# liuzm-slam/VLOAM-NOTED

Measured on NVIDIA B200. Metric: scans/sec, higher is better.
Workload: dtype f32+f64

## Files before the change

vloam-noted_b200/csrc/capi.cu:

```cuda
#include <stdlib.h>
#include <string>
#include <vector>
#include "common.cuh"

static bool g_capture_default = false;
bool vl_debug_capture(const vloam_b200_ctx* c) { return c->h_vScalars && c->h_vScalars[0] != 0; }
int vl_lm_rescan_sorted(vloam_b200_ctx* c);
int vl_solver_trace(vloam_b200_ctx* c, long long* out16);
int vl_lo_trace(vloam_b200_ctx* c, int* out, int n);
int vl_sr_trace(vloam_b200_ctx* c, long long* out, int n);

extern "C" {

void vloam_b200_default_params(vloam_b200_params* p) {
  p->n_scans = 64; p->minimum_range = 5.0f; p->line_res = 0.4f; p->plane_res = 0.8f; p->mapping_skip_frame = 1; p->reserved = 0;
}

const char* vloam_b200_last_error(const vloam_b200_ctx* c) { return c ? c->err : "null context"; }

#define VL_CUDA_CREATE(call)                                                                                       \
  do {                                                                                                             \
    cudaError_t e_ = (call);                                                                                       \
    if (e_ != cudaSuccess) { fprintf(stderr, "vloam_b200_create: %s: %s\n", #call, cudaGetErrorString(e_)); return VLOAM_E_CUDA; } \
  } while (0)

static int alloc_sr_fixed(vloam_b200_ctx* c) {
  const int R = VL_MAX_RINGS, S = VL_MAX_RINGS * VL_SECTORS;
  VL_CUDA_CREATE(cudaEventCreateWithFlags(&c->evSR, cudaEventDisableTiming));
  VL_CUDA_CREATE(cudaEventCreateWithFlags(&c->evSRfeat, cudaEventDisableTiming));
  VL_CUDA_CREATE(cudaMalloc(&c->ringCount, sizeof(int) * R));
  VL_CUDA_CREATE(cudaMalloc(&c->ringStart, sizeof(int) * (R + 1)));
  VL_CUDA_CREATE(cudaMemset(c->ringCount, 0, sizeof(int) * R));
  VL_CUDA_CREATE(cudaMemset(c->ringStart, 0, sizeof(int) * (R + 1)));
  VL_CUDA_CREATE(cudaMalloc(&c->srs, sizeof(SrScalars)));
  VL_CUDA_CREATE(cudaMemset(c->srs, 0, sizeof(SrScalars)));
  VL_CUDA_CREATE(cudaMallocHost(&c->h_srs, sizeof(SrScalars)));
  memset(c->h_srs, 0, sizeof(SrScalars));
  VL_CUDA_CREATE(cudaMalloc(&c->provSharp, sizeof(int) * S * 2));
  VL_CUDA_CREATE(cudaMalloc(&c->provLess, sizeof(int) * S * 20));
  VL_CUDA_CREATE(cudaMalloc(&c->provFlat, sizeof(int) * S * 4));
  int** smalls[] = {&c->cntSharp, &c->cntLess, &c->cntFlat, &c->offSharp, &c->offLess, &c->offFlat};
  for (int** q : smalls) { VL_CUDA_CREATE(cudaMalloc(q, sizeof(int) * S)); VL_CUDA_CREATE(cudaMemset(*q, 0, sizeof(int) * S)); }
  VL_CUDA_CREATE(cudaMalloc(&c->ringDsCount, sizeof(int) * R));
  VL_CUDA_CREATE(cudaMalloc(&c->ringDsOff, sizeof(int) * R));
  c->sr_counts_valid = false; c->n_in = 0; c->nKept = c->nSharp = c->nLessSharp = c->nFlat = c->nLessFlat = 0;
  return VLOAM_OK;
}
static void free_sr_set(vloam_b200_ctx* c) {
  void* dev[] = {c->ringCount, c->ringStart, c->srs, c->provSharp, c->provLess, c->provFlat, c->cntSharp, c->cntLess, c->cntFlat, c->offSharp,
                 c->offLess, c->offFlat, c->ringDsCount, c->ringDsOff, c->in.p, c->ring.p, c->ori.p, c->blockHist.p, c->cloud.p, c->curv.p,
                 c->label.p, c->picked.p, c->sortScratch.p, c->lessFlatProv.p, c->selIdx.p, c->sharp.p, c->flat.p};
  for (void* p : dev) vl_dev_free(c, p);
  if (c->h_srs) cudaFreeHost(c->h_srs);
  if (c->evSR) cudaEventDestroy(c->evSR);
  if (c->evSRfeat) cudaEventDestroy(c->evSRfeat);
}

static int create_impl(vloam_b200_ctx* c, const vloam_b200_params* p, int device);

int vloam_b200_create(const vloam_b200_params* p, int device, vloam_b200_ctx** out) {
  if (!p || !out) return VLOAM_E_INVALID;
  *out = nullptr;
  if (p->n_scans != 16 && p->n_scans != 32 && p->n_scans != 64 && p->n_scans != 128) return VLOAM_E_INVALID;
  if (!(p->line_res >= 0.05f) || !(p->plane_res >= 0.05f) || p->mapping_skip_frame < 1) return VLOAM_E_INVALID;
  if (p->reserved & ~(VLOAM_FLAG_DISTORTION | VLOAM_FLAG_TRANSFORM_TO_END)) return VLOAM_E_INVALID;
  VL_CUDA_CREATE(cudaSetDevice(device));
  vloam_b200_ctx* c = new vloam_b200_ctx();
  const int r = create_impl(c, p, device);
  if (r != VLOAM_OK) { vloam_b200_destroy(c); (void)cudaGetLastError(); return r; }
  *out = c;
  return VLOAM_OK;
}

static int create_impl(vloam_b200_ctx* c, const vloam_b200_params* p, int device) {
  c->prm = *p; c->device = device; c->err[0] = 0; c->launches = 0; c->worker = nullptr; c->timing = false; c->cur = 0;
  c->sr_counts_valid = false; c->n_in = 0; c->lo_inited = false; c->lo_frameCount = 0; c->lm_frameCount = 0; c->lm_optimized = 0; c->skip_frame = false;
  c->nKept = c->nSharp = c->nLessSharp = c->nFlat = c->nLessFlat = 0; c->nCornerLast = c->nSurfLast = 0;
  c->cornerLastPtr = nullptr; c->surfLastPtr = nullptr;
  for (int k = 0; k < 4; ++k) c->dbgLoCost[k] = c->dbgLmCost[k] = 0;
  for (int k = 0; k < 3; ++k) c->stage_ms[k] = 0;
  c->prof_name[0] = 0; c->prof_n = 0; c->prof_created = 0; c->prof_bytes = 0; c->prof_next_bytes = 0;
  {
    const char* e = getenv("VLOAM_ARENA_MB");
    const size_t mb = e ? (size_t)max(atoll(e), 0LL) : 1024;
    c->arena = nullptr; c->arenaCap = 0; c->arenaTop = 0;
    if (mb) { VL_CUDA_CREATE(cudaMalloc(&c->arena, mb << 20)); c->arenaCap = mb << 20; }
  }
  cudaDeviceProp prop;
  VL_CUDA_CREATE(cudaGetDeviceProperties(&prop, device));
  c->num_sms = prop.multiProcessorCount;
  int prLow = 0, prHigh = 0;
  VL_CUDA_CREATE(cudaDeviceGetStreamPriorityRange(&prLow, &prHigh));
  int lv[4] = {2, 1, 2, 2};
  int lvLO = 2;
  if (const char* e = getenv("VLOAM_PRIO")) sscanf(e, "%d,%d,%d,%d,%d", &lv[0], &lv[1], &lv[2], &lv[3], &lvLO);
  if (getenv("VLOAM_NO_PRIORITIES")) lv[0] = lv[1] = lv[2] = lv[3] = lvLO = 0;
  int pr[5];
  for (int k = 0; k < 4; ++k) pr[k] = max(prLow - lv[k], prHigh);
  pr[4] = max(prLow - lvLO, prHigh);
  VL_CUDA_CREATE(cudaStreamCreateWithPriority(&c->stream, cudaStreamNonBlocking, pr[0]));
  VL_CUDA_CREATE(cudaStreamCreateWithPriority(&c->stream2, cudaStreamNonBlocking, pr[1]));
  VL_CUDA_CREATE(cudaStreamCreateWithPriority(&c->stream3, cudaStreamNonBlocking, pr[2]));
  VL_CUDA_CREATE(cudaStreamCreateWithPriority(&c->stream4, cudaStreamNonBlocking, pr[1]));
  VL_CUDA_CREATE(cudaEventCreateWithFlags(&c->evStacksC, cudaEventDisableTiming));
  VL_CUDA_CREATE(cudaStreamCreateWithPriority(&c->streamAux, cudaStreamNonBlocking, pr[2]));
  VL_CUDA_CREATE(cudaEventCreateWithFlags(&c->evAux, cudaEventDisableTiming));
  VL_CUDA_CREATE(cudaEventCreateWithFlags(&c->evAuxZero, cudaEventDisableTiming));
  VL_CUDA_CREATE(cudaEventCreateWithFlags(&c->evUpd, cudaEventDisableTiming));
  VL_CUDA_CREATE(cudaEventCreateWithFlags(&c->evStacks, cudaEventDisableTiming));
  VL_CUDA_CREATE(cudaEventCreateWithFlags(&c->evLast, cudaEventDisableTiming));
  VL_CUDA_CREATE(cudaEventCreateWithFlags(&c->evPose, cudaEventDisableTiming));
  VL_CUDA_CREATE(cudaEventCreateWithFlags(&c->evMap, cudaEventDisableTiming));
  VL_CUDA_CREATE(cudaEventCreateWithFlags(&c->evKeys, cudaEventDisableTiming));
  for (int k = 0; k < 2; ++k) VL_CUDA_CREATE(cudaEventCreateWithFlags(&c->evKeysSel[k], cudaEventDisableTiming));
  c->stacksReady = false; c->lm_reset_pending = true; c->lastSet = 0; c->loGridValid[0] = c->loGridValid[1] = false;
  for (int k = 0; k < 4; ++k) VL_CUDA_CREATE(cudaEventCreate(&c->ev[k]));
  for (int k = 0; k < 12; ++k) { VL_CUDA_CREATE(cudaEventCreate(&c->evx[k])); VL_CUDA_CREATE(cudaEventRecord(c->evx[k], c->stream)); }
  VL_TRY(alloc_sr_fixed(c));
  c->srNext = new SrSet();
  vl_sr_swap(c, *c->srNext);
  { const int r_ = alloc_sr_fixed(c); vl_sr_swap(c, *c->srNext); if (r_ != VLOAM_OK) return r_; }
  c->srNext2 = new SrSet();
  vl_sr_swap(c, *c->srNext2);
  { const int r_ = alloc_sr_fixed(c); vl_sr_swap(c, *c->srNext2); if (r_ != VLOAM_OK) return r_; }
  c->srNextKey = c->srNext2Key = nullptr; c->srNextValid = c->srNext2Valid = false; c->srPendCount = 0;
  VL_CUDA_CREATE(cudaStreamCreateWithPriority(&c->streamSR, cudaStreamNonBlocking, pr[3]));
  VL_CUDA_CREATE(cudaMalloc(&c->los, sizeof(LoScalars)));
  VL_CUDA_CREATE(cudaMalloc(&c->losNext, sizeof(LoScalars)));
  VL_CUDA_CREATE(cudaEventCreateWithFlags(&c->evS2, cudaEventDisableTiming));
  VL_CUDA_CREATE(cudaMallocHost(&c->h_s2flag, 64)); *c->h_s2flag = 0; c->s2seq = 0;
  VL_CUDA_CREATE(cudaEventCreateWithFlags(&c->evLoSolve, cudaEventDisableTiming));
  VL_CUDA_CREATE(cudaEventCreateWithFlags(&c->evLoNext, cudaEventDisableTiming));
  VL_CUDA_CREATE(cudaEventCreateWithFlags(&c->evEnd, cudaEventDisableTiming));
  VL_CUDA_CREATE(cudaStreamCreateWithPriority(&c->streamLO, cudaStreamNonBlocking, pr[4]));
  c->loNextValid = c->loNextQueued = c->srAdopted = c->s2Done = false; c->loAssumeMonotone = c->inProcessFrame = c->loDeferred = false; c->srDeferred = c->sideSubmitted = false; c->preDeferred = c->loPreValid = c->sideWaitsIssued = c->earlyLoArmed = c->stacksAdopted = false; c->loNextSet = 0; c->stackSel = 0; c->stacksNextReady = false;
  VL_CUDA_CREATE(cudaMallocHost(&c->h_los, sizeof(LoScalars)));
  LoScalars hl; memset(&hl, 0, sizeof hl); hl.para_q[3] = 1.0; hl.q_w[3] = 1.0;
  VL_CUDA_CREATE(cudaMemcpy(c->los, &hl, sizeof hl, cudaMemcpyHostToDevice));
  *c->h_los = hl;
  VL_CUDA_CREATE(cudaMalloc(&c->loRingTbl, sizeof(int) * 4 * 160));
  VL_CUDA_CREATE(cudaMalloc(&c->evalOut, sizeof(EvalOut)));
  VL_CUDA_CREATE(cudaMalloc(&c->lms, sizeof(LmSolveState)));
  VL_CUDA_CREATE(cudaMemset(c->lms, 0, sizeof(LmSolveState)));
  VL_CUDA_CREATE(cudaMallocHost(&c->h_lms, sizeof(LmSolveState)));
  VL_CUDA_CREATE(cudaMalloc(&c->lmm, sizeof(LmScalars)));
  VL_CUDA_CREATE(cudaMallocHost(&c->h_lmm, sizeof(LmScalars)));
  memset(c->h_lmm, 0, sizeof(LmScalars));
  VL_CUDA_CREATE(cudaMalloc(&c->cubeC, sizeof(MapCubeTable)));
  VL_CUDA_CREATE(cudaMalloc(&c->cubeS, sizeof(MapCubeTable)));
  VL_CUDA_CREATE(cudaMalloc(&c->vScalars, sizeof(int) * 256));
  VL_CUDA_CREATE(cudaMemset(c->vScalars, 0, sizeof(int) * 256));
  VL_CUDA_CREATE(cudaMallocHost(&c->h_vScalars, sizeof(int) * 256));
  memset(c->h_vScalars, 0, sizeof(int) * 256);
  c->h_vScalars[0] = g_capture_default ? 1 : 0;
  int r = vl_lm_init(c);
  if (r == VLOAM_OK) r = vl_sr_set_attrs(c);
  if (r == VLOAM_OK) r = vl_sort_set_attrs(c);
  if (r == VLOAM_OK) r = vl_solver_set_attrs(c);
  if (r == VLOAM_OK) r = vl_lo_preload(c);
  if (r == VLOAM_OK) r = vl_vg_preload(c);
  if (r == VLOAM_OK) r = vl_lm_preload(c);
  if (r != VLOAM_OK) { fprintf(stderr, "vloam_b200_create: %s\n", c->err); return r; }
  VL_CUDA_CREATE(cudaDeviceSynchronize());
  return VLOAM_OK;
}

void vloam_b200_destroy(vloam_b200_ctx* c) {
  if (!c) return;
  cudaSetDevice(c->device);
  vl_lm_shutdown(c);
  cudaStreamSynchronize(c->stream); cudaStreamSynchronize(c->stream2); cudaStreamSynchronize(c->stream3); cudaStreamSynchronize(c->stream4);
  cudaStreamSynchronize(c->streamSR);
  free_sr_set(c);
  if (c->srNext) { vl_sr_swap(c, *c->srNext); free_sr_set(c); delete c->srNext; c->srNext = nullptr; }
  if (c->srNext2) { vl_sr_swap(c, *c->srNext2); free_sr_set(c); delete c->srNext2; c->srNext2 = nullptr; }
  cudaStreamDestroy(c->streamSR);
  vl_lm_free(c);
  vl_scan_free(&c->loScan[0]); vl_scan_free(&c->loScan[1]);
  if (c->streamLO) { cudaStreamSynchronize(c->streamLO); cudaStreamDestroy(c->streamLO); }
  cudaEventDestroy(c->evS2); cudaEventDestroy(c->evLoSolve); cudaEventDestroy(c->evLoNext); if (c->evEnd) cudaEventDestroy(c->evEnd);
  void* singles[] = {c->los, c->losNext, c->evalOut, c->lms, c->lmm, c->cubeC, c->cubeS, c->vScalars, c->loRingTbl, c->loGridCells[0].p, c->loGridCells[1].p,
                     c->loGridCellOf.p, c->loGridSorted[0].p, c->loGridSorted[1].p, c->dbgLoCorner[0].p, c->dbgLoCorner[1].p, c->dbgLoSurf[0].p,
                     c->dbgLoSurf[1].p, c->dbgKnnIdx[0][0].p, c->dbgKnnIdx[0][1].p, c->dbgKnnIdx[1][0].p, c->dbgKnnIdx[1][1].p, c->dbgKnnD2[0][0].p,
                     c->dbgKnnD2[0][1].p, c->dbgKnnD2[1][0].p, c->dbgKnnD2[1][1].p, c->dbgKnnOk[0][0].p, c->dbgKnnOk[0][1].p, c->dbgKnnOk[1][0].p,
                     c->dbgKnnOk[1][1].p};
  for (void* p : singles) vl_dev_free(c, p);
  void* bufs[] = {c->lessSharp[0].p, c->lessSharp[1].p, c->lessSharp[2].p, c->lessFlat[0].p, c->lessFlat[1].p, c->lessFlat[2].p, c->endSharp[0].p, c->endSharp[1].p, c->endSharp[2].p, c->endFlat[0].p, c->endFlat[1].p, c->endFlat[2].p, c->loCornerIdx.p, c->loSurfIdx.p, c->factors.p, c->factorS.p, c->factorValid.p, c->loFactors.p, c->loFactorValid.p, c->evalPartials.p,
                  c->poolC.p, c->poolS.p, c->stackC.p, c->stackS.p, c->stackCN.p, c->stackSN.p, c->fromMapC.p, c->fromMapS.p, c->knnIdx.p, c->knnD2.p, c->knnOk.p,
                  c->vKeys.p, c->vKeys2.p, c->vHead.p, c->vScan.p, c->vScan2.p, c->vOut.p, c->vIn.p, c->regOut.p, c->tailKeys.p, c->staging.p};
  for (void* p : bufs) vl_dev_free(c, p);
  if (c->h_s2flag) cudaFreeHost(c->h_s2flag);
  cudaFreeHost(c->h_los); cudaFreeHost(c->h_lms); cudaFreeHost(c->h_lmm); cudaFreeHost(c->h_vScalars);
  for (int k = 0; k < 4; ++k) cudaEventDestroy(c->ev[k]);
  for (int k = 0; k < 12; ++k) cudaEventDestroy(c->evx[k]);
  cudaStreamSynchronize(c->stream2); cudaStreamSynchronize(c->stream3);
  cudaEventDestroy(c->evStacks); cudaEventDestroy(c->evLast); cudaEventDestroy(c->evPose); cudaEventDestroy(c->evMap); cudaEventDestroy(c->evKeys); cudaEventDestroy(c->evKeysSel[0]); cudaEventDestroy(c->evKeysSel[1]);
  cudaEventDestroy(c->evStacksC);
  cudaStreamSynchronize(c->streamAux); cudaEventDestroy(c->evAux); cudaEventDestroy(c->evAuxZero); cudaEventDestroy(c->evUpd); cudaStreamDestroy(c->streamAux);
  cudaStreamDestroy(c->stream2); cudaStreamDestroy(c->stream3); cudaStreamDestroy(c->stream4);
  cudaStreamDestroy(c->stream);
  if (c->arena) cudaFree(c->arena);
  delete c;
}

int vloam_b200_begin_frame(vloam_b200_ctx* c) {
  if (!c) return VLOAM_E_INVALID;
  VL_CUDA(cudaSetDevice(c->device));
  c->lm_reset_pending = true;
  return VLOAM_OK;
}

static int register_pending(vloam_b200_ctx* c, const float* key, int n, int stride, bool dev) {
  if (n <= 0 || stride < 3 || !key) { snprintf(c->err, sizeof c->err, "bad cloud shape"); return VLOAM_E_INVALID; }
  if (c->srNextValid && key == c->srNextKey && n == c->srNextN && stride == c->srNextStride) return VLOAM_OK;
  if (c->srNext2Valid && key == c->srNext2Key && n == c->srNext2N && stride == c->srNext2Stride) return VLOAM_OK;
  for (int k = 0; k < c->srPendCount; ++k)
    if (c->srPend[k].key == key && c->srPend[k].n == n && c->srPend[k].stride == stride) return VLOAM_OK;
  if (c->srPendCount == 2) c->srPendCount = 1;
  c->srPend[c->srPendCount].key = key; c->srPend[c->srPendCount].n = n; c->srPend[c->srPendCount].stride = stride; c->srPend[c->srPendCount].dev = dev;
  c->srPendCount++;
  return VLOAM_OK;
}
int vloam_b200_prefetch_scan_device(vloam_b200_ctx* c, const float* d_xyz, int n, int stride) {
  if (!c) return VLOAM_E_INVALID;
  return register_pending(c, d_xyz, n, stride, true);
}
int vloam_b200_prefetch_scan(vloam_b200_ctx* c, const float* xyz, int n, int stride) {
  if (!c) return VLOAM_E_INVALID;
  return register_pending(c, xyz, n, stride, false);
}

int vl_launch_lookahead(vloam_b200_ctx* c) {
  int r = VLOAM_OK;
  while (r == VLOAM_OK && c->srPendCount > 0) {
    const int slot = !c->srNextValid ? 0 : (!c->srNext2Valid ? 1 : -1);
    if (slot < 0) break;
    const vloam_b200_ctx::SrPend pd = c->srPend[0];
    c->srPend[0] = c->srPend[1]; c->srPendCount--;
    SrSet* S = slot ? c->srNext2 : c->srNext;
    const int curNow = c->cur;
    vl_sr_swap(c, *S);
    c->cur = (curNow + slot) % 3;
    vl_tls_stream = c->streamSR;
    if (!c->sideWaitsIssued) cudaStreamWaitEvent(c->streamSR, c->evLoSolve, 0);
    const float* d_xyz = pd.key;
    if (!pd.dev) {
// ... 557 lines not shown
```

vloam-noted_b200/csrc/laser_mapping.cu:

```cuda
#include <limits.h>
#include <float.h>
#include <math_constants.h>
#include <cooperative_groups.h>
#include "common.cuh"
#include "bitonic.cuh"
#include "lm_grid.cuh"
namespace cg = cooperative_groups;
#include <atomic>
#include <chrono>
#include <condition_variable>
#include <functional>
#include <mutex>
#include <thread>

thread_local cudaStream_t vl_tls_stream = nullptr;

struct VlWorker {
  std::thread th;
  std::mutex m;
  std::condition_variable cv;
  std::function<int()> task;
  std::atomic<int> state{0};
  std::atomic<bool> sleeping{false};
  bool quit = false;
// ... 357 lines not shown
    volatile unsigned long long* st = state;
    int excl = 0;
    if (tile > 0) {
      if (lane == 0) st[tile] = tag | (1ull << 32) | (unsigned)tot;
      int look = tile - 1;
      for (;;) {
        const int i0 = look - lane, i1 = look - 32 - lane;
        const unsigned long long w0 = i0 >= 0 ? st[i0] : (tag | (2ull << 32));
        const unsigned long long w1 = i1 >= 0 ? st[i1] : (tag | (2ull << 32));
        const int s0 = (w0 >> 34) == (unsigned long long)epoch ? (int)((w0 >> 32) & 3) : 0;
        const int s1 = (w1 >> 34) == (unsigned long long)epoch ? (int)((w1 >> 32) & 3) : 0;
        const unsigned nr0 = __ballot_sync(0xffffffffu, s0 == 0), in0 = __ballot_sync(0xffffffffu, s0 == 2);
        const unsigned nr1 = __ballot_sync(0xffffffffu, s1 == 0), in1 = __ballot_sync(0xffffffffu, s1 == 2);
        int val; bool done = false; int step = 0;
        if (in0) {
          const int f = __ffs(in0) - 1;
          const unsigned need = f >= 31 ? 0xffffffffu : ((2u << f) - 1u);
          if (nr0 & need) continue;
          val = lane <= f ? (int)(unsigned)w0 : 0; done = true;
        } else {
          if (nr0) continue;
          val = (int)(unsigned)w0; step = 32;
          const int f = in1 ? __ffs(in1) - 1 : 32;
          const unsigned need = f >= 31 ? 0xffffffffu : ((2u << f) - 1u);
          if (!(nr1 & need)) { val += lane <= f ? (int)(unsigned)w1 : 0; step = 64; done = f < 32; }
        }
        for (int d = 16; d > 0; d >>= 1) val += __shfl_xor_sync(0xffffffffu, val, d);
        excl += val;
        if (done) break;
        look -= step;
      }
    }
    if (lane == 0) { st[tile] = tag | (2ull << 32) | (unsigned)(excl + tot); sPrefix = excl; }
  }
  __syncthreads();
  int run = sPrefix + ex;
#pragma unroll
  for (int k = 0; k < 16; ++k) { const int t = v[k]; v[k] = run; run += t; }
  if (base + 15 < n) {
#pragma unroll
    for (int q = 0; q < 4; ++q) *reinterpret_cast<int4*>(out + base + 4 * q) = make_int4(v[4 * q], v[4 * q + 1], v[4 * q + 2], v[4 * q + 3]);
  } else {
#pragma unroll
    for (int k = 0; k < 16; ++k) if (base + k < n) out[base + k] = v[k];
  }
  if (tile == (int)gridDim.x - 1 && threadIdx.x == 0) out[n] = sPrefix + tot;
}
int vl_scan_alloc(VlScan* sc, int n) {
  const int tiles = vl_div_up(n, SCAN_TILE);
  if (sc->state && sc->tiles == tiles) return VLOAM_OK;
  vl_scan_free(sc);
  if (cudaMalloc(&sc->state, sizeof(unsigned long long) * (tiles + 1)) != cudaSuccess) return VLOAM_E_CUDA;
  if (cudaMemset(sc->state, 0, sizeof(unsigned long long) * (tiles + 1)) != cudaSuccess) return VLOAM_E_CUDA;
  if (cudaDeviceSynchronize() != cudaSuccess) return VLOAM_E_CUDA;
  sc->tiles = tiles; sc->epoch = 0;
  return VLOAM_OK;
}
void vl_scan_free(VlScan* sc) { if (sc->state) cudaFree(sc->state); sc->state = nullptr; sc->tiles = 0; }
int vl_scan_exclusive(vloam_b200_ctx* c, const int* in, int n, VlScan* sc, int* out, const int* d_skip) {
  if (!sc->state || sc->tiles != vl_div_up(n, SCAN_TILE) || (((uintptr_t)in | (uintptr_t)out) & 15)) return VLOAM_E_INVALID;
  if (sc->epoch >= (1u << 30) - 1) {
    VL_CUDA(cudaMemsetAsync(sc->state, 0, sizeof(unsigned long long) * (sc->tiles + 1), VL_STREAM(c)));
    sc->epoch = 0;
  }
  ++sc->epoch;
  VL_LAUNCH(lm_scan_chained, sc->tiles, 256, 0, in, n, sc->state, sc->epoch, out, d_skip);
  return VLOAM_OK;
}

__device__ __forceinline__ int lg_cell_of(const float4 p, const float* o) {
  return lm_cell_coord(p.x, o[0], LM_GX) + LM_GX * (lm_cell_coord(p.y, o[1], LM_GY) + LM_GY * lm_cell_coord(p.z, o[2], LM_GZ));
}
__global__ void __launch_bounds__(256) lg_zero(LgGrid g, const LmSub* __restrict__ sub) {
  VL_PDL_WAIT();
  for (int i = blockIdx.x * blockDim.x + threadIdx.x; i < 2 * LM_NCELL; i += gridDim.x * blockDim.x) g.dir[i] = make_int2(0, -1);
  if (blockIdx.x == 0 && threadIdx.x == 0) {
    *g.top = 0;
    LgHeader* h = g.hdr;
    h->valid = 1; h->dirty = 0; h->dead = 0; h->nOps = 0;
    h->cI = sub->cI; h->cJ = sub->cJ; h->cK = sub->cK; h->cenW = sub->cenW; h->cenH = sub->cenH; h->cenD = sub->cenD;
    h->validNum = sub->validNum; h->count[0] = sub->Mc; h->count[1] = sub->Ms;
    for (int k = 0; k < VL_MAX_VALID; ++k) h->validInd[k] = k < sub->validNum ? sub->validInd[k] : 0;
    for (int k = 0; k < 3; ++k) h->origin[k] = sub->gridOrigin[k];
  }
}
__global__ void __launch_bounds__(256) lg_rebuild(LgGrid g, const LmSub* __restrict__ sub, const LmScalars* __restrict__ s, vloam_b200_params prm,
                                                  const MapCubeTable* __restrict__ tc, const MapCubeTable* __restrict__ ts,
                                                  const float4* __restrict__ poolC, const float4* __restrict__ poolS) {
  VL_PDL_WAIT();
  const int nv = sub->validNum, mc = sub->Mc, total = sub->Mc + sub->Ms;
  const float o[3] = {sub->gridOrigin[0], sub->gridOrigin[1], sub->gridOrigin[2]};
  for (int gi = blockIdx.x * blockDim.x + threadIdx.x; gi < total; gi += gridDim.x * blockDim.x) {
    const int kind = gi >= mc;
    const int e = kind ? gi - mc : gi;
    const int* off = sub->gatherOff[kind];
    int lo = 0, hi = nv;
    while (hi - lo > 1) { const int mid = (lo + hi) >> 1; if (off[mid] <= e) lo = mid; else hi = mid; }
    const int cb = sub->validInd[lo];
    const MapCubeTable* tb = kind ? ts : tc;
    const int pos = e - off[lo];
    const float4 p = (kind ? poolS : poolC)[tb->start[cb] + pos];
    unsigned low;
    if (pos >= tb->sorted[cb]) { low = LG_TAIL | (unsigned)pos; g.hdr->dirty = 1; }
    else low = lm_vox_key_cube(p, lm_leaf_inv(prm, kind), cb, s);
    lg_insert(g, kind * LM_NCELL + lg_cell_of(p, o), p, ((unsigned long long)lo << 32) | low, pos);
  }
}

__global__ void __launch_bounds__(256) lm_prepare_fast(LmScalars* __restrict__ s, const LoScalars* __restrict__ lo, RfWork* __restrict__ w,
                                                       LgHeader* __restrict__ gh, int skip, int resetValid, const int* __restrict__ qc = nullptr,
                                                       const int* __restrict__ qs = nullptr, const int* __restrict__ gridTop = nullptr) {
  VL_PDL_WAIT(); vl_chain_stamp(1);
  if (threadIdx.x <= LM_NSEG && !skip) { w->segCount[threadIdx.x] = 0; w->segFill[threadIdx.x] = 0; }
  if (threadIdx.x != 0) return;
  for (int k = 0; k < 4; ++k) s->q_wodom[k] = lo->q_w[k];
  for (int k = 0; k < 3; ++k) s->t_wodom[k] = lo->t_w[k];
  double r[3];
  vl_qrot(s->q_wmap_wodom, s->t_wodom[0], s->t_wodom[1], s->t_wodom[2], r);
  if (skip) {
    vl_qmul(s->q_wmap_wodom, s->q_wodom, s->q_hf);
    for (int k = 0; k < 3; ++k) s->t_hf[k] = r[k] + s->t_wmap_wodom[k];
    return;
  }
  double qn[4];
  vl_qmul(s->q_wmap_wodom, s->q_wodom, qn);
  for (int k = 0; k < 4; ++k) s->pose[k] = qn[k];
  for (int k = 0; k < 3; ++k) s->pose[4 + k] = r[k] + s->t_wmap_wodom[k];
  int cI = (int)((s->pose[4] + 25.0) / 50.0) + s->cenW;
  int cJ = (int)((s->pose[5] + 25.0) / 50.0) + s->cenH;
  int cK = (int)((s->pose[6] + 25.0) / 50.0) + s->cenD;
  if (s->pose[4] + 25.0 < 0) cI--;
  if (s->pose[5] + 25.0 < 0) cJ--;
  if (s->pose[6] + 25.0 < 0) cK--;
  const bool roll = cI < 3 || cI >= VL_CUBE_W - 3 || cJ < 3 || cJ >= VL_CUBE_H - 3 || cK < 3 || cK >= VL_CUBE_D - 3;
  const bool same = gh->valid && !gh->dirty && !roll && resetValid && cI == gh->cI && cJ == gh->cJ && cK == gh->cK && s->cenW == gh->cenW &&
                    s->cenH == gh->cenH && s->cenD == gh->cenD;
  s->needSlow = same ? 0 : 1;
  if (same) { s->validNum = gh->validNum; s->Mc = gh->count[0]; s->Ms = gh->count[1]; gh->nOps = 0; }
  if (qc) {
    s->gridTop = *gridTop; s->gridDirty = gh->dirty; s->gridDead = gh->dead; s->gridCount = gh->count[0] + gh->count[1]; s->gridCountC = gh->count[0];
    s->Qc = *qc; s->Qs = *qs;
    s->optimized = (s->Mc > 10 && s->Ms > 50 && *qc + *qs > 0 && !s->needSlow) ? 1 : 0;
    w->nq = s->optimized ? *qc + *qs : 0;
  }
}

__global__ void __launch_bounds__(256) lg_knn(const LmScalars* __restrict__ s, LgGrid g, const float4* __restrict__ stackC,
                                              const float4* __restrict__ stackS, float4* __restrict__ knnPts, float* __restrict__ knnD2,
                                              unsigned long long* __restrict__ knnKey) {
  VL_PDL_WAIT(); vl_chain_stamp(2);

  const int lane = threadIdx.x & 31;
  const int Qc = s->Qc, Qs = s->Qs, opt = s->optimized;
  double pose[7];
#pragma unroll
  for (int k = 0; k < 7; ++k) pose[k] = s->pose[k];
  const float ox = g.hdr->origin[0], oy = g.hdr->origin[1], oz = g.hdr->origin[2];
  if (!opt) return;
  const int nWarps = (gridDim.x * blockDim.x) >> 5;
  for (int qi = (blockIdx.x * blockDim.x + threadIdx.x) >> 5; qi < Qc + Qs; qi += nWarps) {
    const int kind = qi >= Qc;
    const float4 po = kind ? stackS[qi - Qc] : stackC[qi];
    double r[3];
    vl_qrot(pose, (double)po.x, (double)po.y, (double)po.z, r);
    const float sx = (float)(r[0] + pose[4]), sy = (float)(r[1] + pose[5]), sz = (float)(r[2] + pose[6]);
    const int cx = (int)floorf(__fmul_rn(__fsub_rn(sx, ox), 1.0f / LM_CELL));
    const int cy = (int)floorf(__fmul_rn(__fsub_rn(sy, oy), 1.0f / LM_CELL));
    const int cz = (int)floorf(__fmul_rn(__fsub_rn(sz, oz), 1.0f / LM_CELL));
    float bd[5]; int br[5];
#pragma unroll
    for (int k = 0; k < 5; ++k) { bd[k] = CUDART_INF_F; br[k] = -1; }
    int cnt = 0, head = -1;
    if (lane < 27) {
      const int xx = cx - 1 + lane % 3, yy = cy - 1 + (lane / 3) % 3, zz = cz - 1 + lane / 9;
      if (xx >= 0 && xx < LM_GX && yy >= 0 && yy < LM_GY && zz >= 0 && zz < LM_GZ) {
        const int2 d = g.dir[kind * LM_NCELL + xx + LM_GX * (yy + LM_GY * zz)];
        cnt = d.x; head = d.y;
      }
    }
    while (__any_sync(0xffffffffu, cnt > 0)) {
      const int rb = cnt > 0 ? head * LG_C : 0, rl = min(max(cnt, 0), LG_C);
      VL_WARP_VISIT_FLAT(rb, rl, lane, g.pts, {
        const float d = vl_dist2(sx, sy, sz, t.x, t.y, t.z);
        if (d < bd[4] || (d == bd[4] && d < CUDART_INF_F && lg_key_less(g, p, br[4]))) {
          bd[4] = d; br[4] = p;
#pragma unroll
          for (int k = 4; k > 0; --k)
            if (bd[k] < bd[k - 1] || (bd[k] == bd[k - 1] && lg_key_less(g, br[k], br[k - 1]))) {
              const float td = bd[k]; bd[k] = bd[k - 1]; bd[k - 1] = td;
              const int ti = br[k]; br[k] = br[k - 1]; br[k - 1] = ti;
            }
        }
      });
      cnt -= LG_C;
      if (cnt > 0) head = g.next[head];
    }
    float nd[5]; int nr[5];
#pragma unroll
    for (int k = 0; k < 5; ++k) {
      const unsigned hb = __float_as_uint(bd[0]);
      const unsigned gmin = __reduce_min_sync(0xffffffffu, hb);
      unsigned tie = __ballot_sync(0xffffffffu, hb == gmin && br[0] >= 0);
      int win = -1;
      if (tie) {
        if (__popc(tie) > 1) {
          const unsigned long long ky = (hb == gmin && br[0] >= 0) ? g.key[br[0]] : LG_DEAD;
          const unsigned khi = __reduce_min_sync(0xffffffffu, (unsigned)(ky >> 32));
          const unsigned klo = __reduce_min_sync(0xffffffffu, (unsigned)(ky >> 32) == khi ? (unsigned)ky : 0xffffffffu);
          tie = __ballot_sync(0xffffffffu, ky == (((unsigned long long)khi << 32) | klo));
        }
        win = __ffs(tie) - 1;
      }
      nd[k] = win >= 0 ? __uint_as_float(gmin) : CUDART_INF_F;
      nr[k] = win >= 0 ? __shfl_sync(0xffffffffu, br[0], win) : -1;
      if (lane == win) {
#pragma unroll
        for (int q = 0; q < 4; ++q) { bd[q] = bd[q + 1]; br[q] = br[q + 1]; }
        bd[4] = CUDART_INF_F; br[4] = -1;
      }
    }
#pragma unroll
    for (int k = 0; k < 5; ++k) {
      if (lane == k) {
        knnPts[qi * 5 + k] = nr[k] >= 0 ? g.pts[nr[k]] : make_float4(0.f, 0.f, 0.f, 0.f);
        knnD2[qi * 5 + k] = nd[k];
        if (knnKey) knnKey[qi * 5 + k] = nr[k] >= 0 ? g.key[nr[k]] : LG_DEAD;
      }
    }
  }
}

__global__ void __launch_bounds__(256) lg_keys_to_ids(const unsigned long long* __restrict__ keys, int n, int Qc, const LmSub* __restrict__ sub,
                                                      const LmScalars* __restrict__ s, vloam_b200_params prm, const MapCubeTable* __restrict__ tc,
                                                      const MapCubeTable* __restrict__ ts, const float4* __restrict__ poolC,
                                                      const float4* __restrict__ poolS, int* __restrict__ ids) {
  VL_PDL_WAIT();
  const int t = blockIdx.x * blockDim.x + threadIdx.x;
  if (t >= n) return;
  const unsigned long long key = keys[t];
  if (key == LG_DEAD) { ids[t] = -1; return; }
  const int kind = (t / 5) >= Qc;
  const int slot = (int)(key >> 32);
  const unsigned low = (unsigned)key;
  const int cb = sub->validInd[slot];
  const MapCubeTable* tb = kind ? ts : tc;
  int pos;
  if (low & LG_TAIL) pos = (int)(low & ~LG_TAIL);
  else {
    const float4* pool = (kind ? poolS : poolC) + tb->start[cb];
    const float inv = lm_leaf_inv(prm, kind);
    int lo = 0, hi = tb->sorted[cb];
    while (lo < hi) { const int mid = (lo + hi) >> 1; if (lm_vox_key_cube(pool[mid], inv, cb, s) < low) lo = mid + 1; else hi = mid; }
    pos = lo;
  }
  ids[t] = sub->gatherOff[kind][slot] + pos;
}
__global__ void __launch_bounds__(256) lm_gather(const LmSub* __restrict__ sub, const MapCubeTable* __restrict__ tc, const MapCubeTable* __restrict__ ts,
                                                 const float4* __restrict__ poolC, const float4* __restrict__ poolS, float4* __restrict__ outC,
                                                 float4* __restrict__ outS) {
  VL_PDL_WAIT();
  lm_dev_gather(sub, tc, ts, poolC, poolS, outC, outS);
}

__device__ void lm_sym_eig3(double a[3][3], double evals[3], double evecs[3][3]) {
  double v[3][3] = {{1, 0, 0}, {0, 1, 0}, {0, 0, 1}};
  for (int sweep = 0; sweep < 30; ++sweep) {
    const double off = fabs(a[0][1]) + fabs(a[0][2]) + fabs(a[1][2]);
    if (off == 0.0) break;
    for (int p = 0; p < 2; ++p)
      for (int q = p + 1; q < 3; ++q) {
        if (a[p][q] == 0.0) continue;
        const double theta = (a[q][q] - a[p][p]) / (2.0 * a[p][q]);
        const double t = (theta >= 0 ? 1.0 : -1.0) / (fabs(theta) + sqrt(theta * theta + 1.0));
        const double cs = 1.0 / sqrt(t * t + 1.0), sn = t * cs;
        const double apq = a[p][q];
        a[p][p] -= t * apq;
        a[q][q] += t * apq;
        a[p][q] = a[q][p] = 0.0;
        const int r = 3 - p - q;
        const double arp = a[r][p], arq = a[r][q];
        a[r][p] = a[p][r] = cs * arp - sn * arq;
        a[r][q] = a[q][r] = sn * arp + cs * arq;
        for (int k = 0; k < 3; ++k) {
          const double vkp = v[k][p], vkq = v[k][q];
          v[k][p] = cs * vkp - sn * vkq;
          v[k][q] = sn * vkp + cs * vkq;
        }
      }
  }
  int ord[3] = {0, 1, 2};
  for (int i = 1; i < 3; ++i) for (int j = i; j > 0 && a[ord[j]][ord[j]] < a[ord[j - 1]][ord[j - 1]]; --j) { const int t = ord[j]; ord[j] = ord[j - 1]; ord[j - 1] = t; }
  for (int cidx = 0; cidx < 3; ++cidx) {
    evals[cidx] = a[ord[cidx]][ord[cidx]];
    for (int r = 0; r < 3; ++r) evecs[r][cidx] = v[r][ord[cidx]];
  }
}

__device__ void lm_qr_solve_5x3(double A[5][3], double b[5], double x[3]) {
  int perm[3] = {0, 1, 2};
  double maxpivot = 0.0, diag[3] = {0, 0, 0};
  for (int k = 0; k < 3; ++k) {
    int best = k; double bestn = -1.0;
    for (int j = k; j < 3; ++j) { double n2 = 0; for (int i = k; i < 5; ++i) n2 += A[i][j] * A[i][j]; if (n2 > bestn) { bestn = n2; best = j; } }
    if (best != k) { for (int i = 0; i < 5; ++i) { const double t = A[i][k]; A[i][k] = A[i][best]; A[i][best] = t; } const int t = perm[k]; perm[k] = perm[best]; perm[best] = t; }
    double tail2 = 0; for (int i = k + 1; i < 5; ++i) tail2 += A[i][k] * A[i][k];
    const double c0 = A[k][k];
    double beta, tau, v[5] = {0, 0, 0, 0, 0};
    if (tail2 <= DBL_MIN) { tau = 0; beta = c0; }
    else {
      beta = sqrt(c0 * c0 + tail2);
      if (c0 >= 0) beta = -beta;
      for (int i = k + 1; i < 5; ++i) v[i] = A[i][k] / (c0 - beta);
      tau = (beta - c0) / beta;
    }
    v[k] = 1.0;
    if (tau != 0) {
      for (int j = k + 1; j < 3; ++j) {
        double sm = 0; for (int i = k; i < 5; ++i) sm += v[i] * A[i][j];
        sm *= tau; for (int i = k; i < 5; ++i) A[i][j] -= sm * v[i];
      }
      double sm = 0; for (int i = k; i < 5; ++i) sm += v[i] * b[i];
      sm *= tau; for (int i = k; i < 5; ++i) b[i] -= sm * v[i];
    }
    A[k][k] = beta; for (int i = k + 1; i < 5; ++i) A[i][k] = 0;
    diag[k] = beta;
    if (fabs(beta) > maxpivot) maxpivot = fabs(beta);
  }
  int rank = 0;
  for (int k = 0; k < 3; ++k) if (fabs(diag[k]) > DBL_EPSILON * 3.0 * maxpivot) ++rank;
  double y[3] = {0, 0, 0};
  for (int k = rank - 1; k >= 0; --k) { double sm = b[k]; for (int j = k + 1; j < rank; ++j) sm -= A[k][j] * y[j]; y[k] = sm / A[k][k]; }
  for (int k = 0; k < 3; ++k) x[perm[k]] = y[k];
}

__device__ __forceinline__ bool lm_fit_one(int kind, double P[5][3], double o6[6]) {
  if (!kind) {
    double cen[3] = {0, 0, 0};
    for (int j = 0; j < 5; ++j) for (int k = 0; k < 3; ++k) cen[k] = cen[k] + P[j][k];
    for (int k = 0; k < 3; ++k) cen[k] = cen[k] / 5.0;
    double cov[3][3] = {{0, 0, 0}, {0, 0, 0}, {0, 0, 0}};
    for (int j = 0; j < 5; ++j) {
      const double z[3] = {P[j][0] - cen[0], P[j][1] - cen[1], P[j][2] - cen[2]};
      for (int a = 0; a < 3; ++a) for (int b = 0; b < 3; ++b) cov[a][b] = cov[a][b] + z[a] * z[b];
    }
    double ev[3], evec[3][3];
    lm_sym_eig3(cov, ev, evec);
    if (!(ev[2] > 3 * ev[1])) return false;
    for (int k = 0; k < 3; ++k) { const double u = evec[k][2]; o6[k] = 0.1 * u + cen[k]; o6[3 + k] = -0.1 * u + cen[k]; }
    return true;
  }
  double A[5][3], B[5] = {-1, -1, -1, -1, -1}, nrm[3];
  for (int j = 0; j < 5; ++j) for (int k = 0; k < 3; ++k) A[j][k] = P[j][k];
  lm_qr_solve_5x3(A, B, nrm);
  const double nn = sqrt(nrm[0] * nrm[0] + nrm[1] * nrm[1] + nrm[2] * nrm[2]);
  const double d = 1 / nn;
  if (nn > 0) { nrm[0] /= nn; nrm[1] /= nn; nrm[2] /= nn; }
  for (int j = 0; j < 5; ++j)
    if (fabs(nrm[0] * P[j][0] + nrm[1] * P[j][1] + nrm[2] * P[j][2] + d) > 0.2) return false;
  o6[0] = nrm[0]; o6[1] = nrm[1]; o6[2] = nrm[2]; o6[3] = d; o6[4] = 0; o6[5] = 0;
  return true;
}

__global__ void __launch_bounds__(128) lm_fit(const LmScalars* __restrict__ s, const float4* __restrict__ stackC, const float4* __restrict__ stackS,
                                              const float4* __restrict__ knnPts, const float* __restrict__ knnD2, int* __restrict__ knnOk,
                                              double* __restrict__ factors, int* __restrict__ valid) {
  VL_PDL_WAIT(); vl_chain_stamp(3);

  const int Qc = s->Qc, Qs = s->Qs, opt = s->optimized;
  if (!opt) return;
  for (int qi = blockIdx.x * blockDim.x + threadIdx.x; qi < Qc + Qs; qi += gridDim.x * blockDim.x) {
  const int kind = qi >= Qc;
  const float d4 = knnD2[qi * 5 + 4];
  float4 nb[5];
#pragma unroll
  for (int j = 0; j < 5; ++j) nb[j] = knnPts[qi * 5 + j];
  const float4 po = kind ? stackS[qi - Qc] : stackC[qi];
  bool ok = false;
  double* f = factors + (size_t)qi * 10;
  if ((double)d4 < 1.0) {
    double P[5][3];
#pragma unroll
    for (int j = 0; j < 5; ++j) { const float4 t = nb[j]; P[j][0] = t.x; P[j][1] = t.y; P[j][2] = t.z; }
    double o6[6];
    ok = lm_fit_one(kind, P, o6);
    if (ok) {
      f[0] = kind ? 2.0 : 0.0; f[1] = po.x; f[2] = po.y; f[3] = po.z;
#pragma unroll
      for (int k = 0; k < 6; ++k) f[4 + k] = o6[k];
    }
  }
  valid[qi] = ok ? 1 : 0;
  knnOk[qi] = ok ? 1 : 0;
  }
}

__global__ void __launch_bounds__(128) lm_fit_sets(const float* __restrict__ near, int n, int kind, int* __restrict__ ok, double* __restrict__ prm) {
  VL_PDL_WAIT();
  const int i = blockIdx.x * blockDim.x + threadIdx.x;
  if (i >= n) return;
  double P[5][3], o6[6] = {0, 0, 0, 0, 0, 0};
  for (int j = 0; j < 5; ++j) for (int k = 0; k < 3; ++k) P[j][k] = near[(size_t)i * 15 + j * 3 + k];
  const bool a = lm_fit_one(kind, P, o6);
  ok[i] = a ? 1 : 0;
  for (int k = 0; k < 6; ++k) prm[(size_t)i * 6 + k] = a ? o6[k] : 0.0;
}
int vl_lm_fit_sets(vloam_b200_ctx* c, const float* d_near, int n, int kind, int* d_ok, double* d_prm) {
  VL_LAUNCH(lm_fit_sets, vl_div_up(max(n, 1), 128), 128, 0, d_near, n, kind, d_ok, d_prm);
  VL_CUDA(cudaGetLastError());
  return VLOAM_OK;
}

__global__ void lm_transform_update(LmScalars* s, const LgHeader* __restrict__ gh, const int* __restrict__ gridTop, const LoScalars* __restrict__ los,
                                    LmScalars* hostLmm, LoScalars* hostLos, volatile unsigned* hostFlag, unsigned seq) {
  VL_PDL_WAIT(); vl_chain_stamp(5);
  if (threadIdx.x == 0) {
    if (gh) { s->gridTop = *gridTop; s->gridDirty = gh->dirty; s->gridDead = gh->dead; s->gridCount = gh->count[0] + gh->count[1]; s->gridCountC = gh->count[0]; }
    if (!s->needSlow) {
      const double* q = s->q_wodom;
      const double n2 = q[0] * q[0] + q[1] * q[1] + q[2] * q[2] + q[3] * q[3];
      const double qi[4] = {-q[0] / n2, -q[1] / n2, -q[2] / n2, q[3] / n2};
      vl_qmul(s->pose, qi, s->q_wmap_wodom);
      double r[3];
      vl_qrot(s->q_wmap_wodom, s->t_wodom[0], s->t_wodom[1], s->t_wodom[2], r);
      for (int k = 0; k < 3; ++k) s->t_wmap_wodom[k] = s->pose[4 + k] - r[k];
    }
  }
  if (!hostLmm) return;
  __syncwarp();
  static_assert(sizeof(LmScalars) % 8 == 0 && sizeof(LoScalars) % 8 == 0, "scalar structs are copied as 8-byte words");
  const unsigned long long* a = reinterpret_cast<const unsigned long long*>(s);
  unsigned long long* ha = reinterpret_cast<unsigned long long*>(hostLmm);
  for (int k = threadIdx.x; k < (int)(sizeof(LmScalars) / 8); k += 32) ha[k] = a[k];
  const unsigned long long* b = reinterpret_cast<const unsigned long long*>(los);
  unsigned long long* hb = reinterpret_cast<unsigned long long*>(hostLos);
  for (int k = threadIdx.x; k < (int)(sizeof(LoScalars) / 8); k += 32) hb[k] = b[k];
  __threadfence_system();
  __syncwarp();
  if (threadIdx.x == 0) *hostFlag = seq;
}


__global__ void __launch_bounds__(256) rf_keys(const LmScalars* __restrict__ s, RfWork* __restrict__ w, vloam_b200_params prm,
                                               const MapCubeTable* __restrict__ tc, const MapCubeTable* __restrict__ ts,
                                               const float4* __restrict__ poolC, const float4* __restrict__ poolS,
                                               const float4* __restrict__ stackC, const float4* __restrict__ stackS,
                                               float4* __restrict__ newPts, int* __restrict__ newCube,
                                               unsigned long long* __restrict__ keys, int P, int noTails) {
  VL_PDL_WAIT();

  const int g = blockIdx.x * blockDim.x + threadIdx.x;
  if (g >= P) return;
  const int tailTotal = noTails ? 0 : w->tailOff[LM_NSEG];
  const int Qc = s->Qc, Qs = s->Qs;
  unsigned long long key = ~0ull;
  if (g < tailTotal) {
    int lo = 0, hi = LM_NSEG;
    while (hi - lo > 1) { const int mid = (lo + hi) >> 1; if (w->tailOff[mid] <= g) lo = mid; else hi = mid; }
    const int kind = lo / VL_MAX_VALID, slot = lo % VL_MAX_VALID;
    const int cb = s->validInd[slot];
    const MapCubeTable* t = kind ? ts : tc;
    const int pos = t->sorted[cb] + (g - w->tailOff[lo]);
    const float4 p = (kind ? poolS : poolC)[t->start[cb] + pos];
    const unsigned vk = lm_vox_key_cube(p, lm_leaf_inv(prm, kind), cb, s);
    key = ((unsigned long long)lo << 56) | ((unsigned long long)vk << 26) | (unsigned long long)pos;
  } else if (g < tailTotal + Qc + Qs) {
    const int i = g - tailTotal;
    const int kind = i >= Qc;
    const float4 po = kind ? stackS[i - Qc] : stackC[i];
    double r[3];
    vl_qrot(s->pose, (double)po.x, (double)po.y, (double)po.z, r);
    const float4 p = make_float4((float)(r[0] + s->pose[4]), (float)(r[1] + s->pose[5]), (float)(r[2] + s->pose[6]), po.w);
    const int ci = lm_cube_of(p.x, s->cenW), cj = lm_cube_of(p.y, s->cenH), ck = lm_cube_of(p.z, s->cenD);
    int cb = -1;
    if (ci >= 0 && ci < VL_CUBE_W && cj >= 0 && cj < VL_CUBE_H && ck >= 0 && ck < VL_CUBE_D) cb = ci + VL_CUBE_W * cj + VL_CUBE_W * VL_CUBE_H * ck;
    newPts[i] = p;
    const int slot = cb >= 0 ? w->slotOfCube[cb] : -1;
    newCube[i] = (cb >= 0 && slot < 0) ? cb : -1;
    if (slot >= 0) {
      const unsigned vk = lm_vox_key(p, lm_leaf_inv(prm, kind), ci, cj, ck, s->cenW, s->cenH, s->cenD);
      key = ((unsigned long long)(kind * VL_MAX_VALID + slot) << 56) | ((unsigned long long)vk << 26) | (unsigned long long)((1u << 25) + (unsigned)i);
    }
  }
  keys[g] = key;
  if (key != ~0ull) atomicAdd(&w->segCount[(int)(key >> 56)], 1);
}

__global__ void __launch_bounds__(256) rf_seg_scatter(const unsigned long long* __restrict__ in, int n, RfWork* __restrict__ w,
                                                      unsigned long long* __restrict__ out) {
  VL_PDL_WAIT();

  __shared__ int sb[256];
  __shared__ int sBegin[256];
  const int t = threadIdx.x;
  const int cnt = t < LM_NSEG ? w->segCount[t] : 0;
  int total = 0;
  const int off = lm_scan256(cnt, sb, &total);
  sBegin[t] = off;
  if (blockIdx.x == 0) {
    if (t < LM_NSEG) { w->tailBegin[t] = off; w->firstViolation[t] = INT_MAX; }
    if (t == 0) { w->tailBegin[LM_NSEG] = total; w->nKeysValid = total; }
  }
  __syncthreads();
  const int g = blockIdx.x * blockDim.x + t;
  if (g >= n) return;
  const unsigned long long key = in[g];
  if (key == ~0ull) return;
  const int sg = (int)(key >> 56);
  out[sBegin[sg] + atomicAdd(&w->segFill[sg], 1)] = key;
}
#define RF_SEG_THREADS 512
#define RF_SEG_CAP 8192
__global__ void __launch_bounds__(RF_SEG_THREADS) rf_seg_sort(unsigned long long* __restrict__ keys, const RfWork* __restrict__ w,
                                                              unsigned long long* __restrict__ scratch, int cap) {
  VL_PDL_WAIT();

  extern __shared__ unsigned long long sk[];
  const int sg = blockIdx.x;
  const int beg = w->tailBegin[sg], n = w->tailBegin[sg + 1] - beg;
  if (n <= 1) return;
  int P = 8; while (P < n) P <<= 1;
  if (P <= cap) {
    for (int t = threadIdx.x; t < P; t += RF_SEG_THREADS) sk[t] = t < n ? keys[beg + t] : ~0ull;
    __syncthreads();
    bt_smem_sort<RF_SEG_THREADS>(sk, P);
    for (int t = threadIdx.x; t < n; t += RF_SEG_THREADS) keys[beg + t] = sk[t];
  } else {
    unsigned long long* g = scratch + (size_t)2 * beg;
    for (int t = threadIdx.x; t < P; t += RF_SEG_THREADS) g[t] = t < n ? keys[beg + t] : ~0ull;
    __syncthreads();
    bt_sort_batched<RF_SEG_THREADS>(g, P, 1);
    for (int t = threadIdx.x; t < n; t += RF_SEG_THREADS) keys[beg + t] = g[t];
  }
}

__device__ __forceinline__ float4 rf_key_point(unsigned long long key, const LmScalars* s, const MapCubeTable* tc, const MapCubeTable* ts,
                                               const float4* poolC, const float4* poolS, const float4* newPts) {
  const unsigned ord = (unsigned)(key & 0x3ffffffull);
  if (ord >= (1u << 25)) return newPts[ord - (1u << 25)];
  const int sg = (int)(key >> 56);
  const int kind = sg / VL_MAX_VALID, cb = s->validInd[sg % VL_MAX_VALID];
  return (kind ? poolS : poolC)[(kind ? ts : tc)->start[cb] + (int)ord];
}
#define RF_VOX(key) ((unsigned)(((key) >> 26) & 0x3fffffffull))

__global__ void __launch_bounds__(256) rf_match(const unsigned long long* __restrict__ keys, const LmScalars* __restrict__ s,
                                                const RfWork* __restrict__ w, vloam_b200_params prm, const MapCubeTable* __restrict__ tc,
                                                const MapCubeTable* __restrict__ ts, const float4* __restrict__ poolC,
                                                const float4* __restrict__ poolS, int* __restrict__ unmatchedHead) {
  VL_PDL_WAIT();

  const int t = blockIdx.x * blockDim.x + threadIdx.x;
  if (t >= w->nKeysValid) return;
  const unsigned long long key = keys[t];
  const int sg = (int)(key >> 56);
  const unsigned vk = RF_VOX(key);
  const bool head = (t == w->tailBegin[sg]) || RF_VOX(keys[t - 1]) != vk;
  int um = 0;
  if (head) {
    const int kind = sg / VL_MAX_VALID, cb = s->validInd[sg % VL_MAX_VALID];
    const MapCubeTable* tb = kind ? ts : tc;
// ... 1381 lines not shown
```

Measured before the change: 5500.

## Unroll fit math into registers, add Jacobi early exit, retune stream priorities

```diff
diff --git a/vloam-noted_b200/csrc/capi.cu b/vloam-noted_b200/csrc/capi.cu
--- a/vloam-noted_b200/csrc/capi.cu
+++ b/vloam-noted_b200/csrc/capi.cu
@@ -91,7 +91,7 @@
   c->num_sms = prop.multiProcessorCount;
   int prLow = 0, prHigh = 0;
   VL_CUDA_CREATE(cudaDeviceGetStreamPriorityRange(&prLow, &prHigh));
-  int lv[4] = {2, 1, 2, 2};
+  int lv[4] = {3, 1, 3, 2};
   int lvLO = 2;
   if (const char* e = getenv("VLOAM_PRIO")) sscanf(e, "%d,%d,%d,%d,%d", &lv[0], &lv[1], &lv[2], &lv[3], &lvLO);
   if (getenv("VLOAM_NO_PRIORITIES")) lv[0] = lv[1] = lv[2] = lv[3] = lvLO = 0;
diff --git a/vloam-noted_b200/csrc/laser_mapping.cu b/vloam-noted_b200/csrc/laser_mapping.cu
--- a/vloam-noted_b200/csrc/laser_mapping.cu
+++ b/vloam-noted_b200/csrc/laser_mapping.cu
@@ -533,15 +533,15 @@
 
   const int lane = threadIdx.x & 31;
   const int Qc = s->Qc, Qs = s->Qs, opt = s->optimized;
-  double pose[7];
-#pragma unroll
-  for (int k = 0; k < 7; ++k) pose[k] = s->pose[k];
-  const float ox = g.hdr->origin[0], oy = g.hdr->origin[1], oz = g.hdr->origin[2];
   if (!opt) return;
   const int nWarps = (gridDim.x * blockDim.x) >> 5;
   for (int qi = (blockIdx.x * blockDim.x + threadIdx.x) >> 5; qi < Qc + Qs; qi += nWarps) {
     const int kind = qi >= Qc;
     const float4 po = kind ? stackS[qi - Qc] : stackC[qi];
+    double pose[7];
+#pragma unroll
+    for (int k = 0; k < 7; ++k) pose[k] = s->pose[k];
+    const float ox = g.hdr->origin[0], oy = g.hdr->origin[1], oz = g.hdr->origin[2];
     double r[3];
     vl_qrot(pose, (double)po.x, (double)po.y, (double)po.z, r);
     const float sx = (float)(r[0] + pose[4]), sy = (float)(r[1] + pose[5]), sz = (float)(r[2] + pose[6]);
@@ -643,99 +643,166 @@
   lm_dev_gather(sub, tc, ts, poolC, poolS, outC, outS);
 }
 
-__device__ void lm_sym_eig3(double a[3][3], double evals[3], double evecs[3][3]) {
-  double v[3][3] = {{1, 0, 0}, {0, 1, 0}, {0, 0, 1}};
+#define LM_JACOBI_TOL 1e-20
+
+template <int p, int q>
+__device__ __forceinline__ void lm_jacobi_rot(double (&a)[3][3], double (&v)[3][3]) {
+  if (a[p][q] == 0.0) return;
+  const double theta = (a[q][q] - a[p][p]) / (2.0 * a[p][q]);
+  const double t = (theta >= 0 ? 1.0 : -1.0) / (fabs(theta) + sqrt(theta * theta + 1.0));
+  const double cs = 1.0 / sqrt(t * t + 1.0), sn = t * cs;
+  const double apq = a[p][q];
+  a[p][p] -= t * apq;
+  a[q][q] += t * apq;
+  a[p][q] = a[q][p] = 0.0;
+  constexpr int r = 3 - p - q;
+  const double arp = a[r][p], arq = a[r][q];
+  a[r][p] = a[p][r] = cs * arp - sn * arq;
+  a[r][q] = a[q][r] = sn * arp + cs * arq;
+#pragma unroll
+  for (int k = 0; k < 3; ++k) {
+    const double vkp = v[k][p], vkq = v[k][q];
+    v[k][p] = cs * vkp - sn * vkq;
+    v[k][q] = sn * vkp + cs * vkq;
+  }
+}
+
+template <int i, int j>
+__device__ __forceinline__ void lm_eig_cas(double (&e)[3], double (&v)[3][3]) {
+  if (e[j] < e[i]) {
+    const double t = e[i]; e[i] = e[j]; e[j] = t;
+#pragma unroll
+    for (int r = 0; r < 3; ++r) { const double u = v[r][i]; v[r][i] = v[r][j]; v[r][j] = u; }
+  }
+}
+
+__device__ __forceinline__ void lm_sym_eig3(double (&a)[3][3], double tol, double (&evals)[3], double (&evecs)[3][3]) {
+#pragma unroll
+  for (int r = 0; r < 3; ++r)
+#pragma unroll
+    for (int c = 0; c < 3; ++c) evecs[r][c] = r == c ? 1.0 : 0.0;
   for (int sweep = 0; sweep < 30; ++sweep) {
     const double off = fabs(a[0][1]) + fabs(a[0][2]) + fabs(a[1][2]);
-    if (off == 0.0) break;
-    for (int p = 0; p < 2; ++p)
-      for (int q = p + 1; q < 3; ++q) {
-        if (a[p][q] == 0.0) continue;
-        const double theta = (a[q][q] - a[p][p]) / (2.0 * a[p][q]);
-        const double t = (theta >= 0 ? 1.0 : -1.0) / (fabs(theta) + sqrt(theta * theta + 1.0));
-        const double cs = 1.0 / sqrt(t * t + 1.0), sn = t * cs;
-        const double apq = a[p][q];
-        a[p][p] -= t * apq;
-        a[q][q] += t * apq;
-        a[p][q] = a[q][p] = 0.0;
-        const int r = 3 - p - q;
-        const double arp = a[r][p], arq = a[r][q];
-        a[r][p] = a[p][r] = cs * arp - sn * arq;
-        a[r][q] = a[q][r] = sn * arp + cs * arq;
-        for (int k = 0; k < 3; ++k) {
-          const double vkp = v[k][p], vkq = v[k][q];
-          v[k][p] = cs * vkp - sn * vkq;
-          v[k][q] = sn * vkp + cs * vkq;
-        }
-      }
-  }
-  int ord[3] = {0, 1, 2};
-  for (int i = 1; i < 3; ++i) for (int j = i; j > 0 && a[ord[j]][ord[j]] < a[ord[j - 1]][ord[j - 1]]; --j) { const int t = ord[j]; ord[j] = ord[j - 1]; ord[j - 1] = t; }
-  for (int cidx = 0; cidx < 3; ++cidx) {
-    evals[cidx] = a[ord[cidx]][ord[cidx]];
-    for (int r = 0; r < 3; ++r) evecs[r][cidx] = v[r][ord[cidx]];
-  }
-}
-
-__device__ void lm_qr_solve_5x3(double A[5][3], double b[5], double x[3]) {
+    if (off == 0.0 || off <= tol * (fabs(a[0][0]) + fabs(a[1][1]) + fabs(a[2][2]))) break;
+    lm_jacobi_rot<0, 1>(a, evecs);
+    lm_jacobi_rot<0, 2>(a, evecs);
+    lm_jacobi_rot<1, 2>(a, evecs);
+  }
+#pragma unroll
+  for (int k = 0; k < 3; ++k) evals[k] = a[k][k];
+  lm_eig_cas<0, 1>(evals, evecs);
+  lm_eig_cas<1, 2>(evals, evecs);
+  lm_eig_cas<0, 1>(evals, evecs);
+}
+
+__device__ __forceinline__ void lm_qr_solve_5x3(double (&A)[5][3], double (&b)[5], double (&x)[3]) {
   int perm[3] = {0, 1, 2};
   double maxpivot = 0.0, diag[3] = {0, 0, 0};
+#pragma unroll
   for (int k = 0; k < 3; ++k) {
     int best = k; double bestn = -1.0;
-    for (int j = k; j < 3; ++j) { double n2 = 0; for (int i = k; i < 5; ++i) n2 += A[i][j] * A[i][j]; if (n2 > bestn) { bestn = n2; best = j; } }
-    if (best != k) { for (int i = 0; i < 5; ++i) { const double t = A[i][k]; A[i][k] = A[i][best]; A[i][best] = t; } const int t = perm[k]; perm[k] = perm[best]; perm[best] = t; }
-    double tail2 = 0; for (int i = k + 1; i < 5; ++i) tail2 += A[i][k] * A[i][k];
+#pragma unroll
+    for (int j = k; j < 3; ++j) {
+      double n2 = 0;
+#pragma unroll
+      for (int i = k; i < 5; ++i) n2 += A[i][j] * A[i][j];
+      if (n2 > bestn) { bestn = n2; best = j; }
+    }
+#pragma unroll
+    for (int j = k + 1; j < 3; ++j)
+      if (best == j) {
+#pragma unroll
+        for (int i = 0; i < 5; ++i) { const double t = A[i][k]; A[i][k] = A[i][j]; A[i][j] = t; }
+        const int t = perm[k]; perm[k] = perm[j]; perm[j] = t;
+      }
+    double tail2 = 0;
+#pragma unroll
+    for (int i = k + 1; i < 5; ++i) tail2 += A[i][k] * A[i][k];
     const double c0 = A[k][k];
     double beta, tau, v[5] = {0, 0, 0, 0, 0};
     if (tail2 <= DBL_MIN) { tau = 0; beta = c0; }
     else {
       beta = sqrt(c0 * c0 + tail2);
       if (c0 >= 0) beta = -beta;
+#pragma unroll
       for (int i = k + 1; i < 5; ++i) v[i] = A[i][k] / (c0 - beta);
       tau = (beta - c0) / beta;
     }
     v[k] = 1.0;
     if (tau != 0) {
+#pragma unroll
       for (int j = k + 1; j < 3; ++j) {
-        double sm = 0; for (int i = k; i < 5; ++i) sm += v[i] * A[i][j];
-        sm *= tau; for (int i = k; i < 5; ++i) A[i][j] -= sm * v[i];
+        double sm = 0;
+#pragma unroll
+        for (int i = k; i < 5; ++i) sm += v[i] * A[i][j];
+        sm *= tau;
+#pragma unroll
+        for (int i = k; i < 5; ++i) A[i][j] -= sm * v[i];
       }
-      double sm = 0; for (int i = k; i < 5; ++i) sm += v[i] * b[i];
-      sm *= tau; for (int i = k; i < 5; ++i) b[i] -= sm * v[i];
-    }
-    A[k][k] = beta; for (int i = k + 1; i < 5; ++i) A[i][k] = 0;
+      double sm = 0;
+#pragma unroll
+      for (int i = k; i < 5; ++i) sm += v[i] * b[i];
+      sm *= tau;
+#pragma unroll
+      for (int i = k; i < 5; ++i) b[i] -= sm * v[i];
+    }
+    A[k][k] = beta;
+#pragma unroll
+    for (int i = k + 1; i < 5; ++i) A[i][k] = 0;
     diag[k] = beta;
     if (fabs(beta) > maxpivot) maxpivot = fabs(beta);
   }
   int rank = 0;
+#pragma unroll
   for (int k = 0; k < 3; ++k) if (fabs(diag[k]) > DBL_EPSILON * 3.0 * maxpivot) ++rank;
   double y[3] = {0, 0, 0};
-  for (int k = rank - 1; k >= 0; --k) { double sm = b[k]; for (int j = k + 1; j < rank; ++j) sm -= A[k][j] * y[j]; y[k] = sm / A[k][k]; }
-  for (int k = 0; k < 3; ++k) x[perm[k]] = y[k];
-}
-
-__device__ __forceinline__ bool lm_fit_one(int kind, double P[5][3], double o6[6]) {
+#pragma unroll
+  for (int k = 2; k >= 0; --k)
+    if (k < rank) {
+      double sm = b[k];
+#pragma unroll
+      for (int j = k + 1; j < 3; ++j) if (j < rank) sm -= A[k][j] * y[j];
+      y[k] = sm / A[k][k];
+    }
+#pragma unroll
+  for (int j = 0; j < 3; ++j) x[j] = perm[0] == j ? y[0] : perm[1] == j ? y[1] : y[2];
+}
+
+__device__ __forceinline__ bool lm_fit_one(int kind, double tol, double (&P)[5][3], double (&o6)[6]) {
   if (!kind) {
     double cen[3] = {0, 0, 0};
-    for (int j = 0; j < 5; ++j) for (int k = 0; k < 3; ++k) cen[k] = cen[k] + P[j][k];
+#pragma unroll
+    for (int j = 0; j < 5; ++j)
+#pragma unroll
+      for (int k = 0; k < 3; ++k) cen[k] = cen[k] + P[j][k];
+#pragma unroll
     for (int k = 0; k < 3; ++k) cen[k] = cen[k] / 5.0;
     double cov[3][3] = {{0, 0, 0}, {0, 0, 0}, {0, 0, 0}};
+#pragma unroll
     for (int j = 0; j < 5; ++j) {
       const double z[3] = {P[j][0] - cen[0], P[j][1] - cen[1], P[j][2] - cen[2]};
-      for (int a = 0; a < 3; ++a) for (int b = 0; b < 3; ++b) cov[a][b] = cov[a][b] + z[a] * z[b];
+#pragma unroll
+      for (int a = 0; a < 3; ++a)
+#pragma unroll
+        for (int b = 0; b < 3; ++b) cov[a][b] = cov[a][b] + z[a] * z[b];
     }
     double ev[3], evec[3][3];
-    lm_sym_eig3(cov, ev, evec);
+    lm_sym_eig3(cov, tol, ev, evec);
     if (!(ev[2] > 3 * ev[1])) return false;
+#pragma unroll
     for (int k = 0; k < 3; ++k) { const double u = evec[k][2]; o6[k] = 0.1 * u + cen[k]; o6[3 + k] = -0.1 * u + cen[k]; }
     return true;
   }
   double A[5][3], B[5] = {-1, -1, -1, -1, -1}, nrm[3];
-  for (int j = 0; j < 5; ++j) for (int k = 0; k < 3; ++k) A[j][k] = P[j][k];
+#pragma unroll
+  for (int j = 0; j < 5; ++j)
+#pragma unroll
+    for (int k = 0; k < 3; ++k) A[j][k] = P[j][k];
   lm_qr_solve_5x3(A, B, nrm);
   const double nn = sqrt(nrm[0] * nrm[0] + nrm[1] * nrm[1] + nrm[2] * nrm[2]);
   const double d = 1 / nn;
   if (nn > 0) { nrm[0] /= nn; nrm[1] /= nn; nrm[2] /= nn; }
+#pragma unroll
   for (int j = 0; j < 5; ++j)
     if (fabs(nrm[0] * P[j][0] + nrm[1] * P[j][1] + nrm[2] * P[j][2] + d) > 0.2) return false;
   o6[0] = nrm[0]; o6[1] = nrm[1]; o6[2] = nrm[2]; o6[3] = d; o6[4] = 0; o6[5] = 0;
@@ -763,7 +830,7 @@
 #pragma unroll
     for (int j = 0; j < 5; ++j) { const float4 t = nb[j]; P[j][0] = t.x; P[j][1] = t.y; P[j][2] = t.z; }
     double o6[6];
-    ok = lm_fit_one(kind, P, o6);
+    ok = lm_fit_one(kind, LM_JACOBI_TOL, P, o6);
     if (ok) {
       f[0] = kind ? 2.0 : 0.0; f[1] = po.x; f[2] = po.y; f[3] = po.z;
 #pragma unroll
@@ -775,18 +842,24 @@
   }
 }
 
-__global__ void __launch_bounds__(128) lm_fit_sets(const float* __restrict__ near, int n, int kind, int* __restrict__ ok, double* __restrict__ prm) {
+__global__ void __launch_bounds__(128) lm_fit_sets(const float* __restrict__ near, int n, int kind, double tol, int* __restrict__ ok,
+                                                   double* __restrict__ prm) {
   VL_PDL_WAIT();
   const int i = blockIdx.x * blockDim.x + threadIdx.x;
   if (i >= n) return;
   double P[5][3], o6[6] = {0, 0, 0, 0, 0, 0};
-  for (int j = 0; j < 5; ++j) for (int k = 0; k < 3; ++k) P[j][k] = near[(size_t)i * 15 + j * 3 + k];
-  const bool a = lm_fit_one(kind, P, o6);
+#pragma unroll
+  for (int j = 0; j < 5; ++j)
+#pragma unroll
+    for (int k = 0; k < 3; ++k) P[j][k] = near[(size_t)i * 15 + j * 3 + k];
+  const bool a = lm_fit_one(kind, tol, P, o6);
   ok[i] = a ? 1 : 0;
+#pragma unroll
   for (int k = 0; k < 6; ++k) prm[(size_t)i * 6 + k] = a ? o6[k] : 0.0;
 }
 int vl_lm_fit_sets(vloam_b200_ctx* c, const float* d_near, int n, int kind, int* d_ok, double* d_prm) {
-  VL_LAUNCH(lm_fit_sets, vl_div_up(max(n, 1), 128), 128, 0, d_near, n, kind, d_ok, d_prm);
+  const double tol = getenv("VLOAM_FIT_EXACT_JACOBI") ? 0.0 : LM_JACOBI_TOL;
+  VL_LAUNCH(lm_fit_sets, vl_div_up(max(n, 1), 128), 128, 0, d_near, n, kind, tol, d_ok, d_prm);
   VL_CUDA(cudaGetLastError());
   return VLOAM_OK;
 }
```

After: 5614 (median of 6 runs). 2.1% higher.
